# wazzuck/multimodal-image-transformer

Hardware: AMD Instinct MI355X
Metric: image-caption pairs/sec (train step), 6L/d512 decoder + ViT-B/16, 1/2/4/8 GPU (higher is better)
Workload: dtype bf16; 1 GPU; configs[1]: 6L d512 decoder + ViT-B/16 (197 patches), batch 64/GPU, seq_len 64; global_batch=64, seq_len=64, vocab=10000, memory_mode=patches, parallelism=dp1

## Files before the change

### multimodal-image-transformer_amd/csrc/attention.hip

```cpp
#include "common.h"

namespace {

constexpr int D = 64;

struct AttnK {
  const void* q;
  long q_row, q_batch;
  const void* k;
  long k_row, k_batch;
  const void* v;
  long v_row, v_batch;
  void* o;
  long o_row, o_batch;
  float* lse;
  const int64_t* tok;
  long tok_batch;
  int pad;
  int causal;
  float scale;
  const uint64_t* seed;
  uint32_t site;
  uint32_t thresh;
  float dscale;
// ... 245 lines not shown
  const bf16* Vb = (const bf16*)a.v + b * a.v_batch + h * D;
  const __amdgpu_buffer_rsrc_t rk = __builtin_amdgcn_make_buffer_rsrc((void*)Kb, (short)0, kbytes, 0x00020000);
  const __amdgpu_buffer_rsrc_t rv = __builtin_amdgcn_make_buffer_rsrc((void*)Vb, (short)0, vbytes, 0x00020000);
  bf16x8 qf[2];
  {
    const bf16* Qr = (const bf16*)a.q + b * a.q_batch + h * D + (qlive ? qi : 0) * a.q_row;
#pragma unroll
    for (int kk = 0; kk < 2; ++kk) {
      u32x4 v = *(const u32x4*)(Qr + kk * 32 + g * 8);
      if (!qlive) v = u32x4{0u, 0u, 0u, 0u};
      qf[kk] = __builtin_bit_cast(bf16x8, v);
    }
  }
  const float sl2 = a.scale * 1.4426950408889634f;
  const uint64_t key = a.dropout ? site_key(a.seed, a.site) : 0ull;
  const uint32_t rowbase = ((uint32_t)(b * H + h) * (uint32_t)Lq + (uint32_t)qi) * (uint32_t)Lk + (uint32_t)(g * 4);
  const uint32_t kf = key_fold(key);
  const int64_t* tok = a.tok ? a.tok + b * a.tok_batch : nullptr;
  const int qi32 = (int)qi;

  long kend = Lk;
  if (a.causal) kend = min(Lk, min(Lq, qblk + AQ));
  const int nt = (int)((kend + AK - 1) / AK);

  u32x4 kr[2], vr[2];
  auto gload = [&](long j0) {
#pragma unroll
    for (int i = 0; i < 2; ++i) {
      const int id = tid + 256 * i, r = id >> 3, c = id & 7;
      const long kj = j0 + r;
      const bool ok = kj < Lk;
      kr[i] = __builtin_bit_cast(u32x4, __builtin_amdgcn_raw_buffer_load_b128(
                                            rk, (int)(ok ? (uint32_t)((kj * a.k_row + c * 8) * 2) : A_OOB), 0, 0));
      vr[i] = __builtin_bit_cast(u32x4, __builtin_amdgcn_raw_buffer_load_b128(
                                            rv, (int)(ok ? (uint32_t)((kj * a.v_row + c * 8) * 2) : A_OOB), 0, 0));
    }
  };
  auto lstore = [&](int s) {
    char* Ks = lds + s * (2 * AK * D * 2);
    char* Vs = Ks + AK * D * 2;
#pragma unroll
    for (int i = 0; i < 2; ++i) {
      const int id = tid + 256 * i, r = id >> 3, c = id & 7;
      *(u32x4*)(Ks + koff_k(r, c)) = kr[i];
      *(u32x4*)(Vs + koff_v(r, c * 16)) = vr[i];
    }
  };

  f32x4 ot[4];
#pragma unroll
  for (int i = 0; i < 4; ++i) ot[i] = f32x4{0.f, 0.f, 0.f, 0.f};
  float m = -INFINITY, l = 0.f;

  if (nt > 0) {
    gload(0);
    lstore(0);
  }
  __syncthreads();
  for (int it = 0; it < nt; ++it) {
    const int cur = it & 1;
    const long j0 = (long)it * AK;
    const bool more = it + 1 < nt;
    if (more) gload(j0 + AK);
    const char* Ks = lds + cur * (2 * AK * D * 2);
    const char* Vs = Ks + AK * D * 2;
    f32x4 st[4];
#pragma unroll
    for (int nb = 0; nb < 4; ++nb) st[nb] = f32x4{0.f, 0.f, 0.f, 0.f};
#pragma unroll
    for (int kk = 0; kk < 2; ++kk)
#pragma unroll
      for (int nb = 0; nb < 4; ++nb) {
        const u32x4 kv = *(const u32x4*)(Ks + koff_k(nb * 16 + (lane & 15), kk * 4 + g));
        st[nb] = __builtin_amdgcn_mfma_f32_16x16x32_bf16(__builtin_bit_cast(bf16x8, kv), qf[kk], st[nb], 0, 0, 0);
      }
    uint64_t live;
    {
      const long kj = j0 + lane;
      bool ok = kj < Lk;
      if (ok && tok) ok = tok[kj] != a.pad;
      live = __ballot(ok);
    }
    float s[16];
    float tmax = -INFINITY;
#pragma unroll
    for (int nb = 0; nb < 4; ++nb)
#pragma unroll
      for (int t = 0; t < 4; ++t) {
        const int kb = nb * 16 + g * 4 + t;
        const bool msk = !((live >> kb) & 1ull) | ((a.causal != 0) & ((int)j0 + kb > qi32));
        const float v = msk ? -INFINITY : st[nb][t] * sl2;
        s[nb * 4 + t] = v;
        tmax = fmaxf(tmax, v);
      }
    tmax = fmaxf(tmax, __shfl_xor(tmax, 16, 64));
    tmax = fmaxf(tmax, __shfl_xor(tmax, 32, 64));
    const float mnew = fmaxf(m, tmax);
    const float alpha = (mnew == -INFINITY) ? 1.f : __builtin_amdgcn_exp2f(m - mnew);
    float psum = 0.f;
    float p[16];
#pragma unroll
    for (int k = 0; k < 16; ++k) {
      p[k] = (s[k] == -INFINITY) ? 0.f : __builtin_amdgcn_exp2f(s[k] - mnew);
      psum += p[k];
    }
    psum += __shfl_xor(psum, 16, 64);
    psum += __shfl_xor(psum, 32, 64);
    l = l * alpha + psum;
    m = mnew;
    if (a.dropout) {
#pragma unroll
      for (int nb = 0; nb < 4; ++nb)
#pragma unroll
        for (int t = 0; t < 4; ++t)
          p[nb * 4 + t] *= drop_mul32(kf, rowbase + (uint32_t)(j0 + nb * 16 + t), a.thresh, a.dscale);
    }
#pragma unroll
    for (int i = 0; i < 4; ++i) ot[i] *= alpha;
#pragma unroll
    for (int kk = 0; kk < 2; ++kk) {
      bf16x8 pb;
#pragma unroll
      for (int j = 0; j < 4; ++j) {
        pb[j] = (bf16)p[(2 * kk) * 4 + j];
        pb[4 + j] = (bf16)p[(2 * kk + 1) * 4 + j];
      }
      const int q = (lane & 15) >> 2, pp = lane & 3;
#pragma unroll
      for (int i = 0; i < 4; ++i) {
        const int colb = (i * 16 + 4 * pp) * 2;
        s16x4 lo = __builtin_amdgcn_ds_read_tr16_b64_v4i16(LDS_PTR(s16x4, Vs + koff_v(kk * 32 + g * 4 + q, colb)));
        s16x4 hi = __builtin_amdgcn_ds_read_tr16_b64_v4i16(LDS_PTR(s16x4, Vs + koff_v(kk * 32 + 16 + g * 4 + q, colb)));
        s16x8 vv = {lo[0], lo[1], lo[2], lo[3], hi[0], hi[1], hi[2], hi[3]};
        ot[i] = __builtin_amdgcn_mfma_f32_16x16x32_bf16(__builtin_bit_cast(bf16x8, vv), pb, ot[i], 0, 0, 0);
      }
    }
    if (more) lstore(cur ^ 1);
    __syncthreads();
  }
  if (!qlive) return;
  const float inv = 1.0f / l;
  bf16* O = (bf16*)a.o + b * a.o_batch + qi * a.o_row + h * D;
#pragma unroll
  for (int i = 0; i < 4; ++i) {
    typedef __attribute__((ext_vector_type(4))) __bf16 bf16x4;
    bf16x4 o4 = {(bf16)(ot[i][0] * inv), (bf16)(ot[i][1] * inv), (bf16)(ot[i][2] * inv), (bf16)(ot[i][3] * inv)};
    *(bf16x4*)(O + i * 16 + g * 4) = o4;
  }
  if (a.lse && g == 0) a.lse[(b * H + h) * Lq + qi] = (m + __log2f(l)) * 0.6931471805599453f;
}

constexpr int HK_MAX = 640;
constexpr int HS = 4;

__device__ __forceinline__ float xmax_rows(float v) {
  const auto a = __builtin_amdgcn_permlane16_swap(__float_as_uint(v), __float_as_uint(v), false, false);
  v = __builtin_fmaxf(__uint_as_float(a[0]), __uint_as_float(a[1]));
  const auto b = __builtin_amdgcn_permlane32_swap(__float_as_uint(v), __float_as_uint(v), false, false);
  return __builtin_fmaxf(__uint_as_float(b[0]), __uint_as_float(b[1]));
}
__device__ __forceinline__ float xsum_rows(float v) {
  const auto a = __builtin_amdgcn_permlane16_swap(__float_as_uint(v), __float_as_uint(v), false, false);
  v = __uint_as_float(a[0]) + __uint_as_float(a[1]);
  const auto b = __builtin_amdgcn_permlane32_swap(__float_as_uint(v), __float_as_uint(v), false, false);
  return __uint_as_float(b[0]) + __uint_as_float(b[1]);
}
__device__ __forceinline__ float max16(const float (&s)[16]) {
  const float a = __builtin_fmaxf(__builtin_fmaxf(s[0], s[1]), s[2]), b = __builtin_fmaxf(__builtin_fmaxf(s[3], s[4]), s[5]);
  const float c = __builtin_fmaxf(__builtin_fmaxf(s[6], s[7]), s[8]), d = __builtin_fmaxf(__builtin_fmaxf(s[9], s[10]), s[11]);
  const float e = __builtin_fmaxf(__builtin_fmaxf(s[12], s[13]), s[14]);
  return __builtin_fmaxf(__builtin_fmaxf(__builtin_fmaxf(a, b), c), __builtin_fmaxf(__builtin_fmaxf(d, e), s[15]));
}
constexpr bf16x8 ones8 = {(bf16)1.0f, (bf16)1.0f, (bf16)1.0f, (bf16)1.0f, (bf16)1.0f, (bf16)1.0f, (bf16)1.0f, (bf16)1.0f};

template <bool DROP>
__global__ __attribute__((amdgpu_flat_work_group_size(64, DROP ? 512 : 1024))) void attn_fwd_head(long H, long Lq, long Lk, AttnK a, int kbytes, int vbytes,
                                                      int lkp) {
  extern __shared__ __attribute__((aligned(16))) char lds[];
  char* Ks = lds;
  char* Vs = lds + (long)lkp * 128;
  const int tid = threadIdx.x, lane = tid & 63, w = tid >> 6, g = lane >> 4, nw = blockDim.x >> 6;
  const long h = blockIdx.x, b = blockIdx.y;
  MIT_DASSERT(h < H && Lk <= lkp && lkp <= HK_MAX && Lq > 0);
  const bf16* Kb = (const bf16*)a.k + b * a.k_batch + h * D;
  const bf16* Vb = (const bf16*)a.v + b * a.v_batch + h * D;
  const __amdgpu_buffer_rsrc_t rk = __builtin_amdgcn_make_buffer_rsrc((void*)Kb, (short)0, kbytes, 0x00020000);
  const __amdgpu_buffer_rsrc_t rv = __builtin_amdgcn_make_buffer_rsrc((void*)Vb, (short)0, vbytes, 0x00020000);
  const int nid = lkp * 8;
  for (int base = tid; base < nid; base += HS * (int)blockDim.x) {
    u32x4 kv[HS], vv[HS];
#pragma unroll
    for (int u = 0; u < HS; ++u) {
      const int id = base + u * (int)blockDim.x, r = id >> 3, c = id & 7;
      const bool ok = r < Lk;
      kv[u] = __builtin_bit_cast(u32x4, __builtin_amdgcn_raw_buffer_load_b128(
                                            rk, (int)(ok ? (uint32_t)((r * a.k_row + c * 8) * 2) : A_OOB), 0, 0));
      vv[u] = __builtin_bit_cast(u32x4, __builtin_amdgcn_raw_buffer_load_b128(
                                            rv, (int)(ok ? (uint32_t)((r * a.v_row + c * 8) * 2) : A_OOB), 0, 0));
    }
#pragma unroll
    for (int u = 0; u < HS; ++u) {
      const int id = base + u * (int)blockDim.x, r = id >> 3, c = id & 7;
      if (id < nid) {
        *(u32x4*)(Ks + koff_k(r, c)) = kv[u];
        *(u32x4*)(Vs + koff_v(r, c * 16)) = vv[u];
      }
    }
  }
  __syncthreads();

  const float sl2 = a.scale * 1.4426950408889634f;
  const uint64_t key = DROP ? site_key(a.seed, a.site) : 0ull;
  const int nqt = (int)((Lq + 15) / 16);
  const int q = (lane & 15) >> 2, pp = lane & 3;
  const int kofs = koff_k(lane & 15, g);
  const int kofs1 = koff_k(lane & 15, 4 + g);
  int vofs[4][2];
#pragma unroll
  for (int i = 0; i < 4; ++i) {
    const int colb = (i * 16 + 4 * pp) * 2;
    vofs[i][0] = koff_v(g * 4 + q, colb);
    vofs[i][1] = koff_v(16 + g * 4 + q, colb);
  }
  for (int qt = w; qt < nqt; qt += nw) {
    const long qi = (long)qt * 16 + (lane & 15);
    const bool qlive = qi < Lq;
    bf16x8 qf[2];
    {
      const bf16* Qr = (const bf16*)a.q + b * a.q_batch + h * D + (qlive ? qi : 0) * a.q_row;
#pragma unroll
      for (int kk = 0; kk < 2; ++kk) {
        u32x4 v = *(const u32x4*)(Qr + kk * 32 + g * 8);
        if (!qlive) v = u32x4{0u, 0u, 0u, 0u};
        qf[kk] = __builtin_bit_cast(bf16x8, v);
      }
    }
    const uint32_t rowbase = ((uint32_t)(b * H + h) * (uint32_t)Lq + (uint32_t)qi) * (uint32_t)Lk + (uint32_t)(g * 4);
    const uint32_t kf = key_fold(key);
    f32x4 ot[4];
#pragma unroll
    for (int i = 0; i < 4; ++i) ot[i] = f32x4{0.f, 0.f, 0.f, 0.f};
    float m = -INFINITY, l = 0.f;
    f32x4 lacc = {0.f, 0.f, 0.f, 0.f};
    const char* Kc = Ks;
    const char* Vc = Vs;
    int j0 = 0;
    const int ilk = (int)Lk;
    for (; j0 + 64 <= lkp; j0 += 64, Kc += 64 * 128, Vc += 64 * 128) {
      f32x4 st[4];
#pragma unroll
      for (int nb = 0; nb < 4; ++nb) {
        const u32x4 k0 = *(const u32x4*)(Kc + nb * 2048 + kofs);
        const u32x4 k1 = *(const u32x4*)(Kc + nb * 2048 + kofs1);
        st[nb] = __builtin_amdgcn_mfma_f32_16x16x32_bf16(__builtin_bit_cast(bf16x8, k0), qf[0],
                                                          f32x4{0.f, 0.f, 0.f, 0.f}, 0, 0, 0);
        st[nb] = __builtin_amdgcn_mfma_f32_16x16x32_bf16(__builtin_bit_cast(bf16x8, k1), qf[1], st[nb], 0, 0, 0);
      }
      s16x8 vv[2][4];
#pragma unroll
      for (int hh = 0; hh < 2; ++hh)
#pragma unroll
        for (int i = 0; i < 4; ++i) {
          s16x4 lo = __builtin_amdgcn_ds_read_tr16_b64_v4i16(LDS_PTR(s16x4, Vc + hh * 4096 + vofs[i][0]));
          s16x4 hi = __builtin_amdgcn_ds_read_tr16_b64_v4i16(LDS_PTR(s16x4, Vc + hh * 4096 + vofs[i][1]));
          vv[hh][i] = s16x8{lo[0], lo[1], lo[2], lo[3], hi[0], hi[1], hi[2], hi[3]};
        }
      float s[16];
#pragma unroll
      for (int nb = 0; nb < 4; ++nb)
#pragma unroll
        for (int t = 0; t < 4; ++t) s[nb * 4 + t] = st[nb][t];
      if (__builtin_expect(j0 + 64 > ilk, 0)) {
        const int live = ilk - j0 - g * 4;
#pragma unroll
        for (int k = 0; k < 16; ++k)
          if ((k >> 2) * 16 + (k & 3) >= live) s[k] = -INFINITY;
      }
      float tmax = max16(s);
      tmax = xmax_rows(tmax);
      {
        const float mnew = __builtin_fmaxf(m, tmax * sl2);
        const float alpha = __builtin_amdgcn_exp2f(m - mnew);
        l *= alpha;
        lacc *= alpha;
#pragma unroll
        for (int i = 0; i < 4; ++i) ot[i] *= alpha;
        m = mnew;
      }
      float p[16];
#pragma unroll
      for (int k = 0; k < 16; ++k) p[k] = __builtin_amdgcn_exp2f(fmaf(s[k], sl2, -m));
      if (DROP) {
        float psum = 0.f;
#pragma unroll
        for (int k = 0; k < 16; ++k) psum += p[k];
        l += xsum_rows(psum);
      }
      if (DROP) {
#pragma unroll
        for (int nb = 0; nb < 4; ++nb)
#pragma unroll
          for (int t = 0; t < 4; ++t)
            p[nb * 4 + t] *= drop_mul32(kf, rowbase + (uint32_t)(j0 + nb * 16 + t), a.thresh, a.dscale);
      }
#pragma unroll
      for (int hh = 0; hh < 2; ++hh) {
        bf16x8 pb;
#pragma unroll
        for (int j = 0; j < 8; ++j) pb[j] = (bf16)p[hh * 8 + j];
#pragma unroll
        for (int i = 0; i < 4; ++i)
          ot[i] = __builtin_amdgcn_mfma_f32_16x16x32_bf16(__builtin_bit_cast(bf16x8, vv[hh][i]), pb, ot[i], 0, 0, 0);
        if (!DROP) lacc = __builtin_amdgcn_mfma_f32_16x16x32_bf16(ones8, pb, lacc, 0, 0, 0);
      }
    }
    if (!DROP) l += lacc[0];
    const int ntail = (lkp - j0) >> 4;
    if (ntail) {
      f32x4 st[3];
      float s[12];
#pragma unroll
      for (int nb = 0; nb < 3; ++nb) {
        if (nb < ntail) {
          const u32x4 k0 = *(const u32x4*)(Kc + nb * 2048 + kofs);
          const u32x4 k1 = *(const u32x4*)(Kc + nb * 2048 + kofs1);
          st[nb] = __builtin_amdgcn_mfma_f32_16x16x32_bf16(__builtin_bit_cast(bf16x8, k0), qf[0],
                                                            f32x4{0.f, 0.f, 0.f, 0.f}, 0, 0, 0);
          st[nb] = __builtin_amdgcn_mfma_f32_16x16x32_bf16(__builtin_bit_cast(bf16x8, k1), qf[1], st[nb], 0, 0, 0);
        }
#pragma unroll
        for (int t = 0; t < 4; ++t)
          s[nb * 4 + t] = (nb < ntail && j0 + nb * 16 + g * 4 + t < Lk) ? st[nb][t] : -INFINITY;
      }
      float tmax = s[0];
#pragma unroll
      for (int k = 1; k < 12; ++k) tmax = __builtin_fmaxf(tmax, s[k]);
      tmax = xmax_rows(tmax);
      const float mnew = __builtin_fmaxf(m, tmax * sl2);
      const float alpha = __builtin_amdgcn_exp2f(m - mnew);
      float p[12], psum = 0.f;
#pragma unroll
      for (int k = 0; k < 12; ++k) {
        p[k] = __builtin_amdgcn_exp2f(fmaf(s[k], sl2, -mnew));
        psum += p[k];
      }
      l = l * alpha + xsum_rows(psum);
      m = mnew;
      if (DROP) {
#pragma unroll
        for (int nb = 0; nb < 3; ++nb)
#pragma unroll
          for (int t = 0; t < 4; ++t)
            if (nb < ntail)
              p[nb * 4 + t] *= drop_mul32(kf, rowbase + (uint32_t)(j0 + nb * 16 + t), a.thresh, a.dscale);
// ... 134 lines not shown
#pragma unroll
      for (int t = 0; t < 4; ++t) {
        const long kj = j0 + nb * 16 + g * 4 + t;
        bool msk = !qlive || kj >= Lk || (a.causal && kj > qi);
        if (!msk && tok) msk = tok[kj] == a.pad;
        const float p = msk ? 0.f : exp2f(st[nb][t] * sl2 - lse2);
        const float mul = a.dropout ? drop_mul(key, rowbase + (uint64_t)kj, a.thresh, a.dscale) : 1.f;
        ds[nb * 4 + t] = p * (dp[nb][t] * mul - delta);
      }
#pragma unroll
    for (int kk = 0; kk < 2; ++kk) {
      bf16x8 bs;
#pragma unroll
      for (int j = 0; j < 4; ++j) {
        bs[j] = (bf16)ds[(2 * kk) * 4 + j];
        bs[4 + j] = (bf16)ds[(2 * kk + 1) * 4 + j];
      }
#pragma unroll
      for (int i = 0; i < 4; ++i) dq[i] = __builtin_amdgcn_mfma_f32_16x16x32_bf16(lds_tr_frag(Ks, kk * 32, i * 16, lane), bs,
                                                                              dq[i], 0, 0, 0);
    }
  }
  if (!qlive) return;
  bf16* DQ = (bf16*)gr.dq + b * gr.dq_batch + qi * gr.dq_row + h * D;
  typedef __attribute__((ext_vector_type(4))) __bf16 bf16x4;
#pragma unroll
  for (int i = 0; i < 4; ++i)
    *(bf16x4*)(DQ + i * 16 + g * 4) = bf16x4{(bf16)(dq[i][0] * a.scale), (bf16)(dq[i][1] * a.scale),
                                             (bf16)(dq[i][2] * a.scale), (bf16)(dq[i][3] * a.scale)};
}

__global__ __launch_bounds__(256) void attn_bwd_dkv_mfma(long H, long Lq, long Lk, AttnK a, AttnG gr, AttnBwdBytes nb_) {
  __shared__ __attribute__((aligned(16))) char lds[2 * AQ * D * 2 + 2 * AQ * 4];
  char* Qs = lds;
  char* Ds = lds + AQ * D * 2;
  float* Ls = (float*)(lds + 2 * AQ * D * 2);
  float* Dl = Ls + AQ;
  const int tid = threadIdx.x, lane = tid & 63, w = tid >> 6, g = lane >> 4;
  const long b = blockIdx.z, h = blockIdx.y;
  const long kblk = (long)blockIdx.x * AK;
  const long kl = kblk + w * 16 + (lane & 15);
  const bool klive = kl < Lk;
  const long kr = klive ? kl : 0;
  const bf16* Kr = (const bf16*)a.k + b * a.k_batch + h * D + kr * a.k_row;
  const bf16* Vr = (const bf16*)a.v + b * a.v_batch + h * D + kr * a.v_row;
  bf16x8 kf[2], vf[2];
#pragma unroll
  for (int kk = 0; kk < 2; ++kk) {
    u32x4 k4 = *(const u32x4*)(Kr + kk * 32 + g * 8), v4 = *(const u32x4*)(Vr + kk * 32 + g * 8);
    if (!klive) k4 = v4 = u32x4{0u, 0u, 0u, 0u};
    kf[kk] = __builtin_bit_cast(bf16x8, k4);
    vf[kk] = __builtin_bit_cast(bf16x8, v4);
  }
  const bool kpad = klive && a.tok && a.tok[b * a.tok_batch + kl] == a.pad;
  const float l2e = 1.4426950408889634f;
  const float sl2 = a.scale * l2e;
  const uint64_t key = a.dropout ? site_key(a.seed, a.site) : 0ull;
  const bf16* Qb = (const bf16*)a.q + b * a.q_batch + h * D;
  const bf16* dOb = (const bf16*)gr.dout + b * gr.do_batch + h * D;
  const long bh = b * H + h;
  f32x4 dk[4], dv[4];
#pragma unroll
  for (int i = 0; i < 4; ++i) dk[i] = dv[i] = f32x4{0.f, 0.f, 0.f, 0.f};
  const long qstart = a.causal ? (kblk / AQ) * AQ : 0;
  for (long q0 = qstart; q0 < Lq; q0 += AQ) {
    __syncthreads();
    load_tile_rows(Qs, Qb, a.q_row, q0, Lq, nb_.q, tid);
    load_tile_rows(Ds, dOb, gr.do_row, q0, Lq, nb_.dO, tid);
    if (tid < AQ) {
      const long q = q0 + tid;
      Ls[tid] = q < Lq ? a.lse[bh * Lq + q] * l2e : 0.f;
      Dl[tid] = q < Lq ? gr.delta[bh * Lq + q] : 0.f;
    }
    __syncthreads();
    f32x4 s[4], dp[4];
#pragma unroll
    for (int nb = 0; nb < 4; ++nb) s[nb] = dp[nb] = f32x4{0.f, 0.f, 0.f, 0.f};
#pragma unroll
    for (int kk = 0; kk < 2; ++kk)
#pragma unroll
      for (int nb = 0; nb < 4; ++nb) {
        s[nb] = __builtin_amdgcn_mfma_f32_16x16x32_bf16(lds_row_frag(Qs, nb * 16 + (lane & 15), kk * 4 + g), kf[kk], s[nb],
                                                        0, 0, 0);
        dp[nb] = __builtin_amdgcn_mfma_f32_16x16x32_bf16(lds_row_frag(Ds, nb * 16 + (lane & 15), kk * 4 + g), vf[kk],
                                                         dp[nb], 0, 0, 0);
      }
    float pd[16], ds[16];
#pragma unroll
    for (int nb = 0; nb < 4; ++nb)
#pragma unroll
      for (int t = 0; t < 4; ++t) {
        const int qq = nb * 16 + g * 4 + t;
        const long q = q0 + qq;
        const bool msk = !klive || kpad || q >= Lq || (a.causal && kl > q);
        const float p = msk ? 0.f : exp2f(s[nb][t] * sl2 - Ls[qq]);
        const float mul = a.dropout ? drop_mul(key, ((uint64_t)bh * (uint64_t)Lq + (uint64_t)q) * (uint64_t)Lk + kl, a.thresh,
                                               a.dscale)
                                    : 1.f;
        pd[nb * 4 + t] = p * mul;
        ds[nb * 4 + t] = p * (dp[nb][t] * mul - Dl[qq]);
      }
#pragma unroll
    for (int kk = 0; kk < 2; ++kk) {
      bf16x8 bp, bs;
#pragma unroll
      for (int j = 0; j < 4; ++j) {
        bp[j] = (bf16)pd[(2 * kk) * 4 + j];
        bp[4 + j] = (bf16)pd[(2 * kk + 1) * 4 + j];
        bs[j] = (bf16)ds[(2 * kk) * 4 + j];
        bs[4 + j] = (bf16)ds[(2 * kk + 1) * 4 + j];
      }
#pragma unroll
      for (int i = 0; i < 4; ++i) {
        dv[i] = __builtin_amdgcn_mfma_f32_16x16x32_bf16(lds_tr_frag(Ds, kk * 32, i * 16, lane), bp, dv[i], 0, 0, 0);
        dk[i] = __builtin_amdgcn_mfma_f32_16x16x32_bf16(lds_tr_frag(Qs, kk * 32, i * 16, lane), bs, dk[i], 0, 0, 0);
      }
    }
  }
  if (!klive) return;
  bf16* DK = (bf16*)gr.dk + b * gr.dk_batch + kl * gr.dk_row + h * D;
  bf16* DV = (bf16*)gr.dv + b * gr.dv_batch + kl * gr.dv_row + h * D;
  typedef __attribute__((ext_vector_type(4))) __bf16 bf16x4;
#pragma unroll
  for (int i = 0; i < 4; ++i) {
    *(bf16x4*)(DK + i * 16 + g * 4) = bf16x4{(bf16)(dk[i][0] * a.scale), (bf16)(dk[i][1] * a.scale),
                                             (bf16)(dk[i][2] * a.scale), (bf16)(dk[i][3] * a.scale)};
    *(bf16x4*)(DV + i * 16 + g * 4) = bf16x4{(bf16)dv[i][0], (bf16)dv[i][1], (bf16)dv[i][2], (bf16)dv[i][3]};
  }
}

constexpr int HB_MAXK = 256;
constexpr int HB_NT = 512;
constexpr int HB_SPW = HB_MAXK / 16 / 8;

__global__ __launch_bounds__(512) __attribute__((amdgpu_waves_per_eu(4))) void attn_bwd_head(long H, long Lq, long Lk, AttnK a, AttnG gr, AttnBwdBytes nb_,
                                                        int lkp) {
  extern __shared__ __attribute__((aligned(16))) char lds[];
  char* Ks = lds;
  char* St = Ks + lkp * 128;
  char* Qs = St + lkp * 128;
  char* Ds = Qs + 64 * 128;
  float* Ls = (float*)(Ds + 64 * 128);
  float* Dl = Ls + 64;
  const int tid = threadIdx.x, lane = tid & 63, w = tid >> 6, g = lane >> 4;
  const long h = blockIdx.x, b = blockIdx.y, bh = b * H + h;
  MIT_DASSERT(h < H && Lq <= 64 && Lk <= lkp && lkp <= HB_MAXK);
  const bf16* Qb = (const bf16*)a.q + b * a.q_batch + h * D;
  const bf16* Kb = (const bf16*)a.k + b * a.k_batch + h * D;
  const bf16* Vb = (const bf16*)a.v + b * a.v_batch + h * D;
  const bf16* dOb = (const bf16*)gr.dout + b * gr.do_batch + h * D;
  const bf16* Ob = (const bf16*)a.o + b * a.o_batch + h * D;
  const __amdgpu_buffer_rsrc_t rv = __builtin_amdgcn_make_buffer_rsrc((void*)Vb, (short)0, nb_.v, 0x00020000);
  bf16x8 vf[HB_SPW][2];
#pragma unroll
  for (int si = 0; si < HB_SPW; ++si)
#pragma unroll
    for (int kk = 0; kk < 2; ++kk) {
      const long kl = (w + 8 * si) * 16 + (lane & 15);
      const bool ok = kl < Lk;
      vf[si][kk] = __builtin_bit_cast(
          bf16x8, __builtin_amdgcn_raw_buffer_load_b128(
                      rv, (int)(ok ? (uint32_t)((kl * a.v_row + kk * 32 + g * 8) * 2) : A_OOB), 0, 0));
    }
  {
    const __amdgpu_buffer_rsrc_t rk = __builtin_amdgcn_make_buffer_rsrc((void*)Kb, (short)0, nb_.k, 0x00020000);
    const __amdgpu_buffer_rsrc_t rq = __builtin_amdgcn_make_buffer_rsrc((void*)Qb, (short)0, nb_.q, 0x00020000);
    const __amdgpu_buffer_rsrc_t rd = __builtin_amdgcn_make_buffer_rsrc((void*)dOb, (short)0, nb_.dO, 0x00020000);
    u32x4 kr[4];
#pragma unroll
    for (int i = 0; i < 4; ++i) {
      const int c = tid + HB_NT * i, r = c >> 3, ch = c & 7;
      const bool ok = r < Lk && c < lkp * 8;
      kr[i] = __builtin_bit_cast(u32x4, __builtin_amdgcn_raw_buffer_load_b128(
                                            rk, (int)(ok ? (uint32_t)((r * a.k_row + ch * 8) * 2) : A_OOB), 0, 0));
    }
    const int r = tid >> 3, ch = tid & 7;
    const bool qok = r < Lq;
    const u32x4 qr = __builtin_bit_cast(
        u32x4, __builtin_amdgcn_raw_buffer_load_b128(rq, (int)(qok ? (uint32_t)((r * a.q_row + ch * 8) * 2) : A_OOB), 0, 0));
    const u32x4 dr = __builtin_bit_cast(
        u32x4, __builtin_amdgcn_raw_buffer_load_b128(rd, (int)(qok ? (uint32_t)((r * gr.do_row + ch * 8) * 2) : A_OOB), 0, 0));
    bf16x8 ov = {};
    if (qok) ov = *(const bf16x8*)(Ob + r * a.o_row + ch * 8);
    const float l = (qok && ch == 0) ? a.lse[bh * Lq + r] : 0.f;
#pragma unroll
    for (int i = 0; i < 4; ++i) {
      const int c = tid + HB_NT * i;
      if (c < lkp * 8) *(u32x4*)(Ks + koff_k(c >> 3, c & 7)) = kr[i];
    }
    *(u32x4*)(Qs + koff_k(r, ch)) = qr;
    *(u32x4*)(Ds + koff_k(r, ch)) = dr;
    const bf16x8 dv8 = __builtin_bit_cast(bf16x8, dr);
    float dl = 0.f;
#pragma unroll
    for (int j = 0; j < 8; ++j) dl += (float)dv8[j] * (float)ov[j];
    dl += __shfl_xor(dl, 1, 64);
    dl += __shfl_xor(dl, 2, 64);
    dl += __shfl_xor(dl, 4, 64);
    if (ch == 0) {
      Ls[r] = l * 1.4426950408889634f;
      Dl[r] = dl;
      if (qok) gr.delta[bh * Lq + r] = dl;
    }
  }
  __syncthreads();
  const float sl2 = a.scale * 1.4426950408889634f;
  const uint64_t key = a.dropout ? site_key(a.seed, a.site) : 0ull;
  const int64_t* tok = a.tok ? a.tok + b * a.tok_batch : nullptr;
  typedef __attribute__((ext_vector_type(4))) __bf16 bf16x4;
#pragma unroll
  for (int si = 0; si < HB_SPW; ++si) {
    const int ks = w + 8 * si;
    if (ks * 16 >= lkp) break;
    const int kloc = ks * 16 + (lane & 15);
    const long kl = kloc;
    const bool klive = kl < Lk;
    const bool kpad = klive && tok && tok[kl] == a.pad;
    f32x4 s[4], dp[4];
#pragma unroll
    for (int nb = 0; nb < 4; ++nb) s[nb] = dp[nb] = f32x4{0.f, 0.f, 0.f, 0.f};
#pragma unroll
    for (int kk = 0; kk < 2; ++kk) {
      const bf16x8 kf = lds_row_frag(Ks, kloc, kk * 4 + g);
#pragma unroll
      for (int nb = 0; nb < 4; ++nb) {
        s[nb] = __builtin_amdgcn_mfma_f32_16x16x32_bf16(lds_row_frag(Qs, nb * 16 + (lane & 15), kk * 4 + g), kf, s[nb],
                                                        0, 0, 0);
        dp[nb] = __builtin_amdgcn_mfma_f32_16x16x32_bf16(lds_row_frag(Ds, nb * 16 + (lane & 15), kk * 4 + g), vf[si][kk],
                                                         dp[nb], 0, 0, 0);
      }
    }
    bf16x4 bp4[4], bs4[4];
    const bool kdead = !klive || kpad;
    const uint32_t ilane = ((uint32_t)bh * (uint32_t)Lq + (uint32_t)(g * 4)) * (uint32_t)Lk + (uint32_t)kl;
    const uint32_t kf = key_fold(key);
#pragma unroll
    for (int nb = 0; nb < 4; ++nb) {
      const f32x4 lq4 = *(const f32x4*)(Ls + nb * 16 + g * 4), dl4 = *(const f32x4*)(Dl + nb * 16 + g * 4);
#pragma unroll
      for (int t = 0; t < 4; ++t) {
        const int qq = nb * 16 + g * 4 + t;
        const bool msk = kdead | (qq >= (int)Lq) | ((a.causal != 0) & (kloc > qq));
        const float e = __builtin_amdgcn_exp2f(s[nb][t] * sl2 - lq4[t]);
        const float p = msk ? 0.f : e;
        const float mul =
            a.dropout ? drop_mul32(kf, ilane + (uint32_t)(nb * 16 + t) * (uint32_t)Lk, a.thresh, a.dscale) : 1.f;
        bp4[nb][t] = (bf16)(p * mul);
        bs4[nb][t] = (bf16)(p * (dp[nb][t] * mul - dl4[t]));
      }
      *(bf16x4*)(St + koff_k(kloc, nb * 2 + (g >> 1)) + (g & 1) * 8) = bs4[nb];
    }
    f32x4 dk[4], dv[4];
#pragma unroll
    for (int i = 0; i < 4; ++i) dk[i] = dv[i] = f32x4{0.f, 0.f, 0.f, 0.f};
#pragma unroll
    for (int kk = 0; kk < 2; ++kk) {
      const bf16x8 bp = {bp4[2 * kk][0], bp4[2 * kk][1], bp4[2 * kk][2], bp4[2 * kk][3],
                         bp4[2 * kk + 1][0], bp4[2 * kk + 1][1], bp4[2 * kk + 1][2], bp4[2 * kk + 1][3]};
      const bf16x8 bs = {bs4[2 * kk][0], bs4[2 * kk][1], bs4[2 * kk][2], bs4[2 * kk][3],
                         bs4[2 * kk + 1][0], bs4[2 * kk + 1][1], bs4[2 * kk + 1][2], bs4[2 * kk + 1][3]};
#pragma unroll
      for (int i = 0; i < 4; ++i) {
        dv[i] = __builtin_amdgcn_mfma_f32_16x16x32_bf16(lds_tr_frag(Ds, kk * 32, i * 16, lane), bp, dv[i], 0, 0, 0);
        dk[i] = __builtin_amdgcn_mfma_f32_16x16x32_bf16(lds_tr_frag(Qs, kk * 32, i * 16, lane), bs, dk[i], 0, 0, 0);
      }
    }
    if (klive) {
      bf16* DK = (bf16*)gr.dk + b * gr.dk_batch + kl * gr.dk_row + h * D;
      bf16* DV = (bf16*)gr.dv + b * gr.dv_batch + kl * gr.dv_row + h * D;
#pragma unroll
      for (int i = 0; i < 4; ++i) {
        *(bf16x4*)(DK + i * 16 + g * 4) = bf16x4{(bf16)(dk[i][0] * a.scale), (bf16)(dk[i][1] * a.scale),
                                                 (bf16)(dk[i][2] * a.scale), (bf16)(dk[i][3] * a.scale)};
        *(bf16x4*)(DV + i * 16 + g * 4) = bf16x4{(bf16)dv[i][0], (bf16)dv[i][1], (bf16)dv[i][2], (bf16)dv[i][3]};
      }
    }
  }
  __syncthreads();
  {
    const int qs = w & 3, dh = w >> 2;
    const int qq = qs * 16 + (lane & 15);
    f32x4 dq[2] = {f32x4{0.f, 0.f, 0.f, 0.f}, f32x4{0.f, 0.f, 0.f, 0.f}};
    for (int k0 = 0; k0 < lkp; k0 += 32) {
      const bf16x8 bsf = lds_tr_frag(St, k0, qs * 16, lane);
#pragma unroll
      for (int i = 0; i < 2; ++i)
        dq[i] = __builtin_amdgcn_mfma_f32_16x16x32_bf16(lds_tr_frag(Ks, k0, dh * 32 + i * 16, lane), bsf, dq[i], 0, 0, 0);
    }
    if (qq < Lq) {
      bf16* DQ = (bf16*)gr.dq + b * gr.dq_batch + (long)qq * gr.dq_row + h * D + dh * 32;
#pragma unroll
      for (int i = 0; i < 2; ++i)
        *(bf16x4*)(DQ + i * 16 + g * 4) = bf16x4{(bf16)(dq[i][0] * a.scale), (bf16)(dq[i][1] * a.scale),
                                                 (bf16)(dq[i][2] * a.scale), (bf16)(dq[i][3] * a.scale)};
    }
  }
}

#define DISPATCH_DH(dh, ...)                    \
  do {                                          \
    switch (dh) {                               \
      case 16: { constexpr int DH = 16; __VA_ARGS__; } break;   \
      case 32: { constexpr int DH = 32; __VA_ARGS__; } break;   \
      case 64: { constexpr int DH = 64; __VA_ARGS__; } break;   \
      default: { constexpr int DH = 128; __VA_ARGS__; } break;  \
    }                                           \
  } while (0)

inline bool head_dim_ok(long dh) { return dh == 16 || dh == 32 || dh == 64 || dh == 128; }

AttnK make_k(const mit_attn_args* x) {
  AttnK a;
  a.q = x->q; a.q_row = x->q_row; a.q_batch = x->q_batch;
  a.k = x->k; a.k_row = x->k_row; a.k_batch = x->k_batch;
  a.v = x->v; a.v_row = x->v_row; a.v_batch = x->v_batch;
  a.o = x->o; a.o_row = x->o_row; a.o_batch = x->o_batch;
  a.lse = x->lse; a.tok = x->key_tokens; a.tok_batch = x->tok_batch; a.pad = x->pad_idx;
  a.causal = x->causal; a.scale = x->scale; a.seed = x->seed; a.site = x->site;
  a.dropout = x->drop_p > 0.f;
  a.thresh = drop_threshold(x->drop_p);
  a.dscale = x->drop_p < 1.f ? 1.f / (1.f - x->drop_p) : 0.f;
  return a;
}

}


static double g_idx32_limit = 4294967296.0;
extern "C" int mit_attention_set_index_limit(double limit) {
  g_idx32_limit = limit > 0 ? limit : 4294967296.0;
  return MIT_OK;
}

constexpr int PLAN_SPAN = -1;
struct FwdPlan {
  int family;
  int nw, lkp;
  long kb, vb;
};
struct BwdPlan {
  int family;
  int lkp;
  AttnBwdBytes nb;
};

static FwdPlan plan_fwd(int dtype, long B, long H, long Lq, long Lk, long Dh, const mit_attn_args* x) {
  FwdPlan p{MIT_ATTN_GENERIC, 0, 0, 0, 0};
  const bool mfma_ok = Dh == D && dtype == MIT_BF16 && x->q_row % 8 == 0 && x->q_batch % 8 == 0 && x->k_row % 8 == 0 &&
                       x->k_batch % 8 == 0 && x->v_row % 8 == 0 && x->v_batch % 8 == 0 && x->o_row % 4 == 0 &&
                       x->o_batch % 4 == 0 && ((uintptr_t)x->q | (uintptr_t)x->k | (uintptr_t)x->v) % 16 == 0 &&
                       ((uintptr_t)x->o % 8) == 0;
  if (!mfma_ok) return p;
  p.kb = 2 * ((Lk - 1) * x->k_row + D);
  p.vb = 2 * ((Lk - 1) * x->v_row + D);
  if (p.kb >= (1L << 31) || p.vb >= (1L << 31)) {
    p.family = PLAN_SPAN;
    return p;
  }
  const bool dropout = x->drop_p > 0.f;
  const bool idx32 = !dropout || (double)B * (double)H * (double)Lq * (double)Lk < g_idx32_limit;
  if (!x->causal && !x->key_tokens && Lk <= HK_MAX && H <= 65535 && B <= 65535 && idx32) {
    constexpr int pad = 16;
    p.lkp = (int)((Lk + pad - 1) / pad * pad);
    const int nqt = (int)((Lq + 15) / 16);
    const int maxw = (dropout || 2 * p.lkp * 256 <= 160 * 1024) ? 8 : 16;
    p.nw = std::min(nqt, maxw);
    p.family = dropout ? MIT_ATTN_FWD_HEAD_DROP : MIT_ATTN_FWD_HEAD;
  } else if (idx32) {
    p.family = MIT_ATTN_FWD_MFMA;
  }
  return p;
}

static BwdPlan plan_bwd(int dtype, long B, long H, long Lq, long Lk, long Dh, const mit_attn_args* x,
                        const mit_attn_grads* gg) {
  BwdPlan p{MIT_ATTN_GENERIC, 0, {0, 0, 0, 0}};
  auto al = [](const void* ptr, int n) { return ((uintptr_t)ptr % n) == 0; };
  const bool mfma_ok = Dh == D && dtype == MIT_BF16 && x->q_row % 8 == 0 && x->q_batch % 8 == 0 && x->k_row % 8 == 0 &&
                       x->k_batch % 8 == 0 && x->v_row % 8 == 0 && x->v_batch % 8 == 0 && x->o_row % 8 == 0 &&
                       x->o_batch % 8 == 0 && gg->do_row % 8 == 0 && gg->do_batch % 8 == 0 && gg->dq_row % 4 == 0 &&
                       gg->dq_batch % 4 == 0 && gg->dk_row % 4 == 0 && gg->dk_batch % 4 == 0 && gg->dv_row % 4 == 0 &&
                       gg->dv_batch % 4 == 0 && al(x->q, 16) && al(x->k, 16) && al(x->v, 16) && al(x->o, 16) &&
                       al(gg->dout, 16) && al(gg->dq, 8) && al(gg->dk, 8) && al(gg->dv, 8);
  if (!mfma_ok) return p;
  const long qb = 2 * ((Lq - 1) * x->q_row + D), kb = 2 * ((Lk - 1) * x->k_row + D);
  const long vb = 2 * ((Lk - 1) * x->v_row + D), db = 2 * ((Lq - 1) * gg->do_row + D);
  if (!(qb < (1L << 31) && kb < (1L << 31) && vb < (1L << 31) && db < (1L << 31))) {
    p.family = PLAN_SPAN;
    return p;
  }
  p.nb.q = (int)qb;
  p.nb.k = (int)kb;
  p.nb.v = (int)vb;
  p.nb.dO = (int)db;
  if (Lq <= 64 && Lk <= HB_MAXK && H <= 65535 && B <= 65535 && x->o_row % 8 == 0 &&
      (double)B * (double)H * (double)Lq * (double)Lk < g_idx32_limit) {
    p.lkp = (int)((Lk + 31) / 32 * 32);
    p.family = MIT_ATTN_BWD_HEAD;
  } else {
// ... 105 lines not shown
```

Baseline: 13340 pairs/s.

## Precompute dropout mask bits during backward load phase and deepen forward dropout staging

In the attention backward kernel, the per-element dropout hash is computed up front into a 16-bit mask per key slice while the global loads are in flight, and the main loop reads bits instead of hashing. This hides the hash work behind memory latency. The LSE load is made unconditional so it issues without a branch. The forward kernel with dropout enabled also unrolls its K/V staging loop deeper (8 instead of 4) to keep more loads outstanding. Costs are extra registers for mbits and kv staging, which can lower occupancy.

Result: faster. 13470 pairs/s (median of 6 runs) (+1.0%).

```diff
diff --git a/multimodal-image-transformer_amd/csrc/attention.hip b/multimodal-image-transformer_amd/csrc/attention.hip
--- a/multimodal-image-transformer_amd/csrc/attention.hip
+++ b/multimodal-image-transformer_amd/csrc/attention.hip
@@ -421,6 +421,7 @@
 
 constexpr int HK_MAX = 640;
 constexpr int HS = 4;
+constexpr int HS_DROP = 8;
 
 __device__ __forceinline__ float xmax_rows(float v) {
   const auto a = __builtin_amdgcn_permlane16_swap(__float_as_uint(v), __float_as_uint(v), false, false);
@@ -448,6 +449,7 @@
   extern __shared__ __attribute__((aligned(16))) char lds[];
   char* Ks = lds;
   char* Vs = lds + (long)lkp * 128;
+  constexpr int HSN = DROP ? HS_DROP : HS;
   const int tid = threadIdx.x, lane = tid & 63, w = tid >> 6, g = lane >> 4, nw = blockDim.x >> 6;
   const long h = blockIdx.x, b = blockIdx.y;
   MIT_DASSERT(h < H && Lk <= lkp && lkp <= HK_MAX && Lq > 0);
@@ -456,10 +458,10 @@
   const __amdgpu_buffer_rsrc_t rk = __builtin_amdgcn_make_buffer_rsrc((void*)Kb, (short)0, kbytes, 0x00020000);
   const __amdgpu_buffer_rsrc_t rv = __builtin_amdgcn_make_buffer_rsrc((void*)Vb, (short)0, vbytes, 0x00020000);
   const int nid = lkp * 8;
-  for (int base = tid; base < nid; base += HS * (int)blockDim.x) {
-    u32x4 kv[HS], vv[HS];
-#pragma unroll
-    for (int u = 0; u < HS; ++u) {
+  for (int base = tid; base < nid; base += HSN * (int)blockDim.x) {
+    u32x4 kv[HSN], vv[HSN];
+#pragma unroll
+    for (int u = 0; u < HSN; ++u) {
       const int id = base + u * (int)blockDim.x, r = id >> 3, c = id & 7;
       const bool ok = r < Lk;
       kv[u] = __builtin_bit_cast(u32x4, __builtin_amdgcn_raw_buffer_load_b128(
@@ -468,7 +470,7 @@
                                             rv, (int)(ok ? (uint32_t)((r * a.v_row + c * 8) * 2) : A_OOB), 0, 0));
     }
 #pragma unroll
-    for (int u = 0; u < HS; ++u) {
+    for (int u = 0; u < HSN; ++u) {
       const int id = base + u * (int)blockDim.x, r = id >> 3, c = id & 7;
       if (id < nid) {
         *(u32x4*)(Ks + koff_k(r, c)) = kv[u];
@@ -909,6 +911,7 @@
   const bf16* Ob = (const bf16*)a.o + b * a.o_batch + h * D;
   const __amdgpu_buffer_rsrc_t rv = __builtin_amdgcn_make_buffer_rsrc((void*)Vb, (short)0, nb_.v, 0x00020000);
   bf16x8 vf[HB_SPW][2];
+  uint32_t mbits[HB_SPW] = {};
 #pragma unroll
   for (int si = 0; si < HB_SPW; ++si)
 #pragma unroll
@@ -939,7 +942,22 @@
         u32x4, __builtin_amdgcn_raw_buffer_load_b128(rd, (int)(qok ? (uint32_t)((r * gr.do_row + ch * 8) * 2) : A_OOB), 0, 0));
     bf16x8 ov = {};
     if (qok) ov = *(const bf16x8*)(Ob + r * a.o_row + ch * 8);
-    const float l = (qok && ch == 0) ? a.lse[bh * Lq + r] : 0.f;
+    const float l = a.lse[bh * Lq + (qok ? r : 0)];
+    if (a.dropout) {
+      const uint32_t kf = key_fold(site_key(a.seed, a.site));
+#pragma unroll
+      for (int si = 0; si < HB_SPW; ++si) {
+        const uint32_t i0 = ((uint32_t)bh * (uint32_t)Lq + (uint32_t)(g * 4)) * (uint32_t)Lk +
+                            (uint32_t)((w + 8 * si) * 16 + (lane & 15));
+        uint32_t bits = 0;
+        if ((w + 8 * si) * 16 < lkp) {
+#pragma unroll
+          for (int k = 0; k < 16; ++k)
+            bits |= (uint32_t)(lowbias32((i0 + (uint32_t)((k >> 2) * 16 + (k & 3)) * (uint32_t)Lk) ^ kf) >= a.thresh) << k;
+        }
+        mbits[si] = bits;
+      }
+    }
 #pragma unroll
     for (int i = 0; i < 4; ++i) {
       const int c = tid + HB_NT * i;
@@ -955,14 +973,13 @@
     dl += __shfl_xor(dl, 2, 64);
     dl += __shfl_xor(dl, 4, 64);
     if (ch == 0) {
-      Ls[r] = l * 1.4426950408889634f;
+      Ls[r] = qok ? l * 1.4426950408889634f : 0.f;
       Dl[r] = dl;
       if (qok) gr.delta[bh * Lq + r] = dl;
     }
   }
   __syncthreads();
   const float sl2 = a.scale * 1.4426950408889634f;
-  const uint64_t key = a.dropout ? site_key(a.seed, a.site) : 0ull;
   const int64_t* tok = a.tok ? a.tok + b * a.tok_batch : nullptr;
   typedef __attribute__((ext_vector_type(4))) __bf16 bf16x4;
 #pragma unroll
@@ -989,8 +1006,6 @@
     }
     bf16x4 bp4[4], bs4[4];
     const bool kdead = !klive || kpad;
-    const uint32_t ilane = ((uint32_t)bh * (uint32_t)Lq + (uint32_t)(g * 4)) * (uint32_t)Lk + (uint32_t)kl;
-    const uint32_t kf = key_fold(key);
 #pragma unroll
     for (int nb = 0; nb < 4; ++nb) {
       const f32x4 lq4 = *(const f32x4*)(Ls + nb * 16 + g * 4), dl4 = *(const f32x4*)(Dl + nb * 16 + g * 4);
@@ -1000,8 +1015,7 @@
         const bool msk = kdead | (qq >= (int)Lq) | ((a.causal != 0) & (kloc > qq));
         const float e = __builtin_amdgcn_exp2f(s[nb][t] * sl2 - lq4[t]);
         const float p = msk ? 0.f : e;
-        const float mul =
-            a.dropout ? drop_mul32(kf, ilane + (uint32_t)(nb * 16 + t) * (uint32_t)Lk, a.thresh, a.dscale) : 1.f;
+        const float mul = a.dropout ? ((mbits[si] >> (nb * 4 + t)) & 1u ? a.dscale : 0.f) : 1.f;
         bp4[nb][t] = (bf16)(p * mul);
         bs4[nb][t] = (bf16)(p * (dp[nb][t] * mul - dl4[t]));
       }
```
